# hamorrar/juicefs

Hardware: AMD Instinct MI355X
Metric: sealed+checksummed GB/s, 4 MiB blocks (higher is better)
Workload: dtype u8; 1 GPU; 64.0 GiB device-resident batch of 4 MiB blocks per GPU, aes256gcm seal + CRC32C full; blocks_per_gpu=16384, resident_blocks_per_gpu=16384, block_bytes=4194304, algo=aes256gcm, mode=seal, aes_kernel=ttable, engine=one process per GPU, parallelism=block-sharded x1, no collective

## Files before the change

### juicefs_amd/csrc/jfsx_dev.h

```cpp
#pragma once
#include "jfsx_internal.h"

namespace jfsx {

__device__ __forceinline__ uint32_t lds_u32(const char *lds, uint32_t byteaddr) {
    return *reinterpret_cast<const uint32_t *>(lds + byteaddr);
}
__device__ __forceinline__ uint4 lds_u4(const char *lds, uint32_t byteaddr) {
    return *reinterpret_cast<const uint4 *>(lds + byteaddr);
}

template <int K>
__device__ __forceinline__ uint32_t byte_x4(uint32_t x) {
    uint32_t r;
    if constexpr (K == 0)
        asm("v_lshlrev_b32_sdwa %0, 2, %1 dst_sel:DWORD dst_unused:UNUSED_PAD src0_sel:DWORD src1_sel:BYTE_0" : "=v"(r) : "v"(x));
    else if constexpr (K == 1)
        asm("v_lshlrev_b32_sdwa %0, 2, %1 dst_sel:DWORD dst_unused:UNUSED_PAD src0_sel:DWORD src1_sel:BYTE_1" : "=v"(r) : "v"(x));
    else if constexpr (K == 2)
        asm("v_lshlrev_b32_sdwa %0, 2, %1 dst_sel:DWORD dst_unused:UNUSED_PAD src0_sel:DWORD src1_sel:BYTE_2" : "=v"(r) : "v"(x));
    else
        asm("v_lshlrev_b32_sdwa %0, 2, %1 dst_sel:DWORD dst_unused:UNUSED_PAD src0_sel:DWORD src1_sel:BYTE_3" : "=v"(r) : "v"(x));
    return r;
}
#define CRC_T(t, x, k) lds_u32(lds, byte_x4<(k)>(x) + CB + 1024u * (t))

template <uint32_t CB, int S = 16>
__device__ __forceinline__ uint32_t crc_piece(const char *lds, uint32_t A, uint32_t p0, uint32_t p1, uint32_t p2,
                                              uint32_t p3) {
#define X3(a, b, c) __builtin_amdgcn_bitop3_b32((a), (b), (c), 0x96)
    uint32_t s = S < 0 ? A : X3(CRC_T(S, A, 0), CRC_T(S + 1, A, 1), CRC_T(S + 2, A, 2)) ^ CRC_T(S + 3, A, 3);
    uint32_t q = p0 ^ s;
    return X3(X3(X3(CRC_T(0, q, 0), CRC_T(1, q, 1), CRC_T(2, q, 2)), X3(CRC_T(3, q, 3), CRC_T(4, p1, 0), CRC_T(5, p1, 1)),
                 X3(CRC_T(6, p1, 2), CRC_T(7, p1, 3), CRC_T(8, p2, 0))),
              X3(CRC_T(9, p2, 1), CRC_T(10, p2, 2), CRC_T(11, p2, 3)),
              X3(CRC_T(12, p3, 0), CRC_T(13, p3, 1), X3(CRC_T(14, p3, 2), CRC_T(15, p3, 3), 0u)));
#undef X3
}

typedef __attribute__((address_space(1))) const uint32_t gcu32;
struct CrcL1Base {
    uint64_t a, b;
};
__device__ __forceinline__ CrcL1Base crc_l1_base(const uint32_t *gcrc) {
    CrcL1Base g = {(uint64_t)gcrc + 8192u, (uint64_t)gcrc + 12288u};
    asm volatile("" : "+s"(g.a), "+s"(g.b));
    return g;
}
template <int I>
__device__ __forceinline__ uint32_t crc_l1_term(const CrcL1Base &g, uint4 p) {
    const uint32_t w = I < 4 ? p.y : (I < 8 ? p.z : p.w);
    const uint32_t o = byte_x4<(I & 3)>(w);
    const __attribute__((address_space(1))) char *t = (const __attribute__((address_space(1))) char *)(I < 8 ? g.a : g.b);
    return *(gcu32 *)(t + o + (1024 * (4 + I) - (I < 8 ? 8192 : 12288)));
}

template <int S, int LG, int UR, int J = 0>
__device__ __forceinline__ void crc_l1_issue(const CrcL1Base &g, const uint4 (&d)[UR], uint32_t (&lv)[LG]) {
    if constexpr (J < LG) {
        lv[J] = crc_l1_term<LG * (S / UR) + J>(g, d[S % UR]);
        crc_l1_issue<S, LG, UR, J + 1>(g, d, lv);
    }
}

constexpr uint32_t kCrcbXl = 16 * 256;
__device__ __forceinline__ const uint32_t *crc_composed(const DevTables &tab) { return tab.crcx + kCrcxDwords; }
__device__ __forceinline__ uint32_t crc_xlb(const DevTables &tab, uint32_t l) {
    const uint32_t *b = crc_composed(tab) + kCrcbXl;
    asm volatile("" : "+s"(b));
    return b[l];
}
__device__ __forceinline__ uint32_t crc_xl(const DevTables &tab, uint32_t l) {
    const uint32_t *x = tab.crcx;
    asm volatile("" : "+s"(x));
    return x[l];
}
template <uint32_t CB>
__device__ __forceinline__ uint32_t crc_piece_b(const char *lds, uint32_t B, uint32_t p0, uint32_t L) {
    const uint32_t q = p0 ^ B;
    return __builtin_amdgcn_bitop3_b32(
        __builtin_amdgcn_bitop3_b32(CRC_T(0, q, 0), CRC_T(1, q, 1), CRC_T(2, q, 2), 0x96), CRC_T(3, q, 3), L, 0x96);
}
template <uint32_t CB>
__device__ __forceinline__ uint32_t crc_shift1008(const char *lds, uint32_t A) {
    return __builtin_amdgcn_bitop3_b32(CRC_T(16, A, 0), CRC_T(17, A, 1), CRC_T(18, A, 2), 0x96) ^ CRC_T(19, A, 3);
}

template <int CRCMODE>
__device__ __forceinline__ uint4 crc_src(uint4 c, uint4 p) {
    return (CRCMODE & 4) ? c : p;
}

template <uint32_t CB, int S = 16>
__device__ __noinline__ uint32_t crc_partial(const char *lds, uint32_t A, const uint32_t p[4], int n) {
    uint32_t c = S < 0 ? A : CRC_T(S, A, 0) ^ CRC_T(S + 1, A, 1) ^ CRC_T(S + 2, A, 2) ^ CRC_T(S + 3, A, 3);
    for (int i = 0; i < n; i++) {
        uint32_t byte = (p[i >> 2] >> (8 * (i & 3))) & 0xffu;
        c = lds_u32(lds, (((c ^ byte) & 0xffu) << 2) + CB + 1024u * 15) ^ (c >> 8);
    }
    return c;
}

typedef unsigned int v4u __attribute__((ext_vector_type(4)));
typedef __attribute__((address_space(1))) v4u gv4u;
__device__ __forceinline__ uint4 gld16(const uint8_t *p) {
    const v4u v = *(const gv4u *)(p);
    return make_uint4(v.x, v.y, v.z, v.w);
}
__device__ __forceinline__ uint4 gld16_nt(const uint8_t *p) {
    const v4u v = __builtin_nontemporal_load((const gv4u *)(p));
    return make_uint4(v.x, v.y, v.z, v.w);
}
__device__ __forceinline__ void gst16(uint8_t *p, uint4 v) {
    v4u w = {v.x, v.y, v.z, v.w};
    *(gv4u *)(p) = w;
}
__device__ __forceinline__ void gst16_nt(uint8_t *p, uint4 v) {
    v4u w = {v.x, v.y, v.z, v.w};
    __builtin_nontemporal_store(w, (gv4u *)(p));
}
template <int NT>
__device__ __forceinline__ uint4 ald16(const uint8_t *p) { return (NT & 1) ? gld16_nt(p) : gld16(p); }
template <int NT>
__device__ __forceinline__ void ast16(uint8_t *p, uint4 v) {
    if (NT & 2)
        gst16_nt(p, v);
    else
        gst16(p, v);
}

__device__ __forceinline__ uint4 load_piece(const uint8_t *src, uint64_t o, uint64_t end) {
    if (o + 16 <= end) return gld16(src + o);
    uint32_t w[4] = {0, 0, 0, 0};
    for (uint64_t i = o; i < end && i < o + 16; i++) w[(i - o) >> 2] |= (uint32_t)src[i] << (8 * ((i - o) & 3));
    return make_uint4(w[0], w[1], w[2], w[3]);
}

__device__ __forceinline__ void store_piece(uint8_t *dst, uint64_t o, uint64_t end, uint4 v) {
    if (o + 16 <= end) {
        gst16(dst + o, v);
        return;
    }
    uint32_t w[4] = {v.x, v.y, v.z, v.w};
    for (uint64_t i = o; i < end && i < o + 16; i++) dst[i] = (uint8_t)(w[(i - o) >> 2] >> (8 * ((i - o) & 3)));
}


__device__ __forceinline__ void crc_verify_block(const BlkDev &blk, BlkOut &o, uint32_t lane) {
    const uint64_t nseg = (blk.len + kSeg - 1) / kSeg;
    for (uint64_t base = 0; base < nseg; base += 64) {
        const uint64_t s = base + lane;
        bool bad = false;
        uint32_t got = 0, ex = 0;
        if (s < nseg) {
            got = blk.crc_calc[s];
            const uint8_t *e = blk.crc + 4 * s;
            ex = ((uint32_t)e[0] << 24) | ((uint32_t)e[1] << 16) | ((uint32_t)e[2] << 8) | e[3];
            bad = got != ex;
        }
        const uint64_t m = __ballot(bad);
        if (m) {
            const int first = __builtin_ctzll(m);
            const uint32_t g2 = __shfl(got, first, 64), e2 = __shfl(ex, first, 64);
            if (lane == 0) {
                o.bad_seg = (int32_t)(base + first);
                o.got = g2;
                o.expect = e2;
            }
            return;
        }
    }
}

}
```

### juicefs_amd/csrc/jfsx_gcm.hip

```cpp

#include "jfsx_dev.h"

#define JFSX_HD __device__ __forceinline__
#define BS3(a, b, c, tt) __builtin_amdgcn_bitop3_b32((a), (b), (c), (tt))
#define PERM(hi, lo, sel) __builtin_amdgcn_perm((hi), (lo), (sel))
#define OPAQUE(x)                                 \
    do {                                          \
        (x) = __builtin_amdgcn_readfirstlane(x);  \
        asm volatile("" : "+s"(x));               \
    } while (0)
#include "jfsx_aes_bs.h"

namespace jfsx {

constexpr int kAeadNt = 3;
constexpr uint32_t kLdsCrc = 0;
constexpr uint32_t kLdsTT = 20480;
constexpr uint32_t kLdsGh = 24576;
constexpr uint32_t kLdsAesOff = 24576;
constexpr uint32_t kLdsAes = 65536 + kLdsAesOff;
constexpr uint32_t kLdsBasis = kLdsAes + 65536;
constexpr uint32_t kLdsSegRaw = kLdsBasis + 2048;
constexpr uint32_t kLdsSegFlag = kLdsSegRaw + 512;
constexpr uint32_t kLdsP = kLdsSegFlag + 512;
constexpr uint32_t kLdsBytes = kLdsP + 4096 + 32;

__device__ __forceinline__ uint32_t rotl8(uint32_t x) { return __builtin_amdgcn_alignbit(x, x, 24); }
__device__ __forceinline__ uint32_t xor3(uint32_t a, uint32_t b, uint32_t c) {
    return __builtin_amdgcn_bitop3_b32(a, b, c, 0x96);
}
__device__ __forceinline__ uint32_t rk_load(const uint32_t *rk, int i) {
    uint32_t k = rk[i];
    if (i >= 8 && i < 56) {
        k = (k >> 8) | (k << 24);
        OPAQUE(k);
    }
    return k;
}

#define AES_SEL(k) (0x0c020000u | ((4u + (k)) << 8))
#define TA(w, k) lds_u32(lds, __builtin_amdgcn_perm((w), loff, AES_SEL(k)) + kLdsAesOff)
#define TB(w, k) lds_u32(lds, __builtin_amdgcn_perm((w), loff, AES_SEL(k)) + (kLdsAesOff + 128u))

#define AES_COL(o, i0, i1, i2, i3, rkv) \
    o = xor3(TA(i0, 0), TB(i2, 2), rotl8(xor3(TA(i1, 1), TB(i3, 3), (rkv))));
#define AES_ROUND(o0, o1, o2, o3, i0, i1, i2, i3, r) \
    AES_COL(o0, i0, i1, i2, i3, rk[4 * (r) + 0])     \
    AES_COL(o1, i1, i2, i3, i0, rk[4 * (r) + 1])     \
    AES_COL(o2, i2, i3, i0, i1, rk[4 * (r) + 2])     \
    AES_COL(o3, i3, i0, i1, i2, rk[4 * (r) + 3])

#define AES_LAST(o, a, b, c, d, rkv)                                                             \
    o = __builtin_amdgcn_bitop3_b32(                                                             \
            __builtin_amdgcn_bitop3_b32(TB(a, 0), TA(b, 1), 0xffu, 0xe4) ,       \
            __builtin_amdgcn_bitop3_b32(TA(c, 2), TB(d, 3), 0x00ff0000u, 0xe4),                 \
            0x0000ffffu, 0xe4) ^ (rkv);

template <int NS>
__device__ __forceinline__ void aes_ctr_blocks(const char *lds, uint32_t loff, const uint32_t *rk, const uint32_t *k1,
                                               const uint32_t (&ctr)[NS], uint32_t (&ks)[NS][4]) {
    uint32_t a[NS][4], b[NS][4];
#pragma unroll
    for (int s = 0; s < NS; s++) {
        const uint32_t x3 = __builtin_bswap32(ctr[s]) ^ rk[3];
        a[s][0] = k1[0] ^ rotl8(TB(x3, 3));
        a[s][1] = k1[1] ^ TB(x3, 2);
        a[s][2] = k1[2] ^ rotl8(TA(x3, 1));
        a[s][3] = k1[3] ^ TA(x3, 0);
    }
#pragma unroll
    for (int r = 2; r <= 13; r += 2) {
#pragma unroll
        for (int s = 0; s < NS; s++) { AES_ROUND(b[s][0], b[s][1], b[s][2], b[s][3], a[s][0], a[s][1], a[s][2], a[s][3], r); }
#pragma unroll
        for (int s = 0; s < NS; s++) { AES_ROUND(a[s][0], a[s][1], a[s][2], a[s][3], b[s][0], b[s][1], b[s][2], b[s][3], r + 1); }
    }
#pragma unroll
    for (int s = 0; s < NS; s++) {
        AES_LAST(ks[s][0], a[s][0], a[s][1], a[s][2], a[s][3], rk[56]);
        AES_LAST(ks[s][1], a[s][1], a[s][2], a[s][3], a[s][0], rk[57]);
        AES_LAST(ks[s][2], a[s][2], a[s][3], a[s][0], a[s][1], rk[58]);
        AES_LAST(ks[s][3], a[s][3], a[s][0], a[s][1], a[s][2], rk[59]);
    }
}

__device__ __forceinline__ void aes_r2_uniform(const char *lds, uint32_t loff, const uint32_t *rk, const uint32_t *k1,
                                               uint32_t U, uint32_t (&u)[4]) {
    const uint32_t x3 = __builtin_bswap32(U << 8) ^ rk[3];
    const uint32_t a1 = k1[1] ^ TB(x3, 2);
    const uint32_t a2 = k1[2] ^ rotl8(TA(x3, 1));
    const uint32_t a3 = k1[3] ^ TA(x3, 0);
    u[0] = xor3(TB(a2, 2), rotl8(xor3(TA(a1, 1), TB(a3, 3), rk[8])), 0u);
    u[1] = xor3(TA(a1, 0), TB(a3, 2), rotl8(TA(a2, 1) ^ rk[9]));
    u[2] = xor3(TA(a2, 0), rotl8(xor3(TA(a3, 1), TB(a1, 3), rk[10])), 0u);
    u[3] = xor3(TA(a3, 0), TB(a1, 2), rotl8(TB(a2, 3) ^ rk[11]));
}

__device__ __forceinline__ uint4 aes_r2_entry(const char *lds, uint32_t loff, uint32_t rk3, uint32_t k10, uint32_t c) {
    const uint32_t x3 = (c << 24) ^ rk3;
    const uint32_t a0 = k10 ^ rotl8(TB(x3, 3));
    return make_uint4(TA(a0, 0), rotl8(TB(a0, 3)), TB(a0, 2), rotl8(TA(a0, 1)));
}

template <int I>
struct AesStep {
    static constexpr int value = I;
};
struct AesNoSide {
    template <int I>
    __device__ __forceinline__ void operator()(AesStep<I>) const {}
};
template <int NS, class Side>
__device__ __forceinline__ void aes_rounds_3_14(const char *lds, uint32_t loff, const uint32_t *rk,
                                                uint32_t (&b)[NS][4], uint32_t (&ks)[NS][4], const Side &side) {
    uint32_t a[NS][4];
    side(AesStep<0>());
#pragma unroll
    for (int s = 0; s < NS; s++) { AES_ROUND(a[s][0], a[s][1], a[s][2], a[s][3], b[s][0], b[s][1], b[s][2], b[s][3], 3); }
    side(AesStep<1>());
#define JFSX_AES_PAIR(r)                                                                                                \
    _Pragma("unroll") for (int s = 0; s < NS; s++) {                                                                    \
        AES_ROUND(b[s][0], b[s][1], b[s][2], b[s][3], a[s][0], a[s][1], a[s][2], a[s][3], r);                           \
    }                                                                                                                   \
    side(AesStep<(r) - 2>());                                                                                           \
    _Pragma("unroll") for (int s = 0; s < NS; s++) {                                                                    \
        AES_ROUND(a[s][0], a[s][1], a[s][2], a[s][3], b[s][0], b[s][1], b[s][2], b[s][3], (r) + 1);                     \
    }                                                                                                                   \
    side(AesStep<(r) - 1>());
    JFSX_AES_PAIR(4)
    JFSX_AES_PAIR(6)
    JFSX_AES_PAIR(8)
    JFSX_AES_PAIR(10)
    JFSX_AES_PAIR(12)
#undef JFSX_AES_PAIR
#pragma unroll
    for (int s = 0; s < NS; s++) {
        AES_LAST(ks[s][0], a[s][0], a[s][1], a[s][2], a[s][3], 0u);
        AES_LAST(ks[s][1], a[s][1], a[s][2], a[s][3], a[s][0], 0u);
        AES_LAST(ks[s][2], a[s][2], a[s][3], a[s][0], a[s][1], 0u);
        AES_LAST(ks[s][3], a[s][3], a[s][0], a[s][1], a[s][2], 0u);
    }
}

template <int NS, class Side = AesNoSide>
__device__ __forceinline__ void aes_ctr_blocks_u(const char *lds, uint32_t loff, const uint32_t *rk,
                                                 const uint32_t *k1, const uint32_t (&ctr)[NS],
                                                 const uint32_t (&u)[NS][4], const uint32_t (&du)[NS][4],
                                                 const uint32_t (&cym)[NS], uint32_t (&ks)[NS][4],
                                                 const Side &side = Side()) {
    uint32_t b[NS][4];
#define UC(t, w) (__builtin_amdgcn_bitop3_b32((t), cym[s], du[s][w], 0x78) ^ u[s][w])
#pragma unroll
    for (int s = 0; s < NS; s++) {
        const uint4 pe = lds_u4(lds, ((ctr[s] << 4) & 0xff0u) + kLdsP);
        b[s][0] = UC(pe.x, 0);
        b[s][1] = UC(pe.y, 1);
        b[s][2] = UC(pe.z, 2);
        b[s][3] = UC(pe.w, 3);
    }
#undef UC
    aes_rounds_3_14<NS>(lds, loff, rk, b, ks, side);
}

template <int Q, class Side>
__device__ __forceinline__ void aes_ctr_blocks_p(const char *lds, uint32_t loff, const uint32_t *rk, uint32_t pb,
                                                 const uint32_t (&u)[4], const uint32_t (&du)[4], uint32_t cy3,
                                                 uint32_t (&ks)[2][4], const Side &side) {
    uint32_t b[2][4];
#pragma unroll
    for (int s = 0; s < 2; s++) {
        const uint4 pe = lds_u4(lds, pb + 1024u * (Q + s));
        const uint32_t t[4] = {pe.x, pe.y, pe.z, pe.w};
#pragma unroll
        for (int w = 0; w < 4; w++)
            b[s][w] = Q + s == 3 ? __builtin_amdgcn_bitop3_b32(t[w], cy3, du[w], 0x78) ^ u[w] : t[w] ^ u[w];
    }
    aes_rounds_3_14<2>(lds, loff, rk, b, ks, side);
}

struct GhLane {
    uint32_t sel[4];
    uint32_t off[4];
    bool r1, r2;
    uint32_t p1, p2;
};

__device__ __forceinline__ GhLane gh_lane(uint32_t lane) {
    GhLane g;
    const uint32_t q = lane & 15, k = q >> 2;
#pragma unroll
    for (int bb = 0; bb < 4; bb++) g.sel[bb] = 0x0c0c0000u | ((4u + ((bb + q) & 3)) << 8) | (uint32_t)bb;
#pragma unroll
    for (int dd = 0; dd < 4; dd++) {
        uint32_t o = 0;
#pragma unroll
        for (int bb = 0; bb < 4; bb++) {
            const uint32_t j = 4 * ((dd + k) & 3) + ((bb + q) & 3);
            o |= (j << 4) << (8 * bb);
        }
        g.off[dd] = o;
    }
    g.r1 = (k & 1) != 0;
    g.r2 = (k & 2) != 0;
    g.p1 = g.r1 ? 0x07060504u : 0x03020100u;
    g.p2 = g.r2 ? 0x07060504u : 0x03020100u;
    return g;
}

__device__ __forceinline__ void gh_rho(const uint32_t a[4], const GhLane &g, uint32_t R[4]) {
    uint32_t u[4];
#pragma unroll
    for (int i = 0; i < 4; i++) u[i] = PERM(a[(i + 2) & 3], a[i], g.p2);
#pragma unroll
    for (int i = 0; i < 4; i++) R[i] = PERM(u[(i + 1) & 3], u[i], g.p1);
}
__device__ __forceinline__ void gh_rho_inv(const uint32_t R[4], const GhLane &g, uint32_t a[4]) {
    uint32_t u[4];
#pragma unroll
    for (int i = 0; i < 4; i++) u[i] = g.r1 ? R[(i + 3) & 3] : R[i];
#pragma unroll
    for (int i = 0; i < 4; i++) a[i] = g.r2 ? u[(i + 2) & 3] : u[i];
}

__device__ __forceinline__ void ghash_step(const char *lds, uint32_t R[4], const GhLane &g, uint4 c) {
#if JFSX_GH8 == 4
    uint32_t S[4] = {c.x, c.y, c.z, c.w};
#pragma unroll
    for (int h = 0; h < 4; h++) {
        uint4 t[4];
#pragma unroll
        for (int q = 0; q < 4; q++) t[q] = lds_u4(lds, kLdsGh + __builtin_amdgcn_perm(R[h], g.off[h], g.sel[q]));
#define GX(f, i) S[i] = xor3(xor3(t[0].f, t[1].f, t[2].f), t[3].f, S[i])
        GX(x, 0); GX(y, 1); GX(z, 2); GX(w, 3);
#undef GX
        __builtin_amdgcn_sched_barrier(0);
    }
#elif JFSX_GH8
    uint32_t S[4] = {c.x, c.y, c.z, c.w};
#pragma unroll
    for (int h = 0; h < 2; h++) {
        uint4 t[8];
#pragma unroll
        for (int q = 0; q < 8; q++) {
            const int dd = 2 * h + (q >> 2), bb = q & 3;
            t[q] = lds_u4(lds, kLdsGh + __builtin_amdgcn_perm(R[dd], g.off[dd], g.sel[bb]));
        }
#define GX(f, i) S[i] = xor3(xor3(t[0].f, t[1].f, t[2].f), xor3(t[3].f, t[4].f, t[5].f), xor3(t[6].f, t[7].f, S[i]))
        GX(x, 0); GX(y, 1); GX(z, 2); GX(w, 3);
#undef GX
        __builtin_amdgcn_sched_barrier(0);
    }
#else
    uint4 t[16];
#pragma unroll
    for (int dd = 0; dd < 4; dd++)
#pragma unroll
        for (int bb = 0; bb < 4; bb++)
            t[4 * dd + bb] = lds_u4(lds, kLdsGh + __builtin_amdgcn_perm(R[dd], g.off[dd], g.sel[bb]));
#define GX(f, cf) xor3(xor3(xor3(t[0].f, t[1].f, t[2].f), xor3(t[3].f, t[4].f, t[5].f), xor3(t[6].f, t[7].f, t[8].f)), \
                       xor3(t[9].f, t[10].f, t[11].f), xor3(xor3(t[12].f, t[13].f, t[14].f), t[15].f, cf))
    const uint32_t S[4] = {GX(x, c.x), GX(y, c.y), GX(z, c.z), GX(w, c.w)};
#undef GX
#endif
    gh_rho(S, g, R);
}

struct Stream {
    uint64_t sub0, sub1;
    uint32_t acc[4];
    uint64_t jlast;
    bool has;
    uint32_t A, lend;
    uint64_t seg0;
};

__device__ __forceinline__ void crc_share(char *lds, uint32_t slot, uint32_t raw) {
    atomicXor(reinterpret_cast<uint32_t *>(lds + kLdsSegRaw) + slot, raw);
    reinterpret_cast<uint32_t *>(lds + kLdsSegFlag)[slot] = 1u;
}

template <int CRCMODE>
__device__ __forceinline__ void crc_segment_done(const BlkDev &blk, const DevTables &tab, uint32_t lane, uint32_t xl,
                                                 uint64_t seg0, uint32_t A, bool partial, char *lds, uint64_t c0) {
    const uint32_t raw = wave_xor(crc_mulmod(xl, A));
    if (lane == 0) {
        if (partial) {
            crc_share(lds, (uint32_t)((seg0 - c0) / kSeg), raw);
            return;
        }
        const uint32_t crc = ~(tab.crcx[96] ^ raw);
        const uint64_t si = seg0 / kSeg;
        if ((CRCMODE & 3) == 1)
            *reinterpret_cast<uint32_t *>(blk.crc + 4 * si) = __builtin_bswap32(crc);
        else
            blk.crc_calc[si] = crc;
    }
}

template <int CRCMODE>
__device__ __noinline__ void crc_segment_end(const BlkDev &blk, const DevTables &tab, uint32_t lane, uint32_t xl,
                                             uint64_t seg0, uint64_t seg1, uint32_t A, uint32_t lend,
                                             uint64_t tailRef, bool partial, char *lds, uint32_t slot) {
    const uint32_t Lseg = (uint32_t)(seg1 - seg0);
    uint32_t v;
    if (lend == 0) {
        const uint32_t sh = tailRef == seg1 ? xl : crc_mulmod(crc_xpow8_fast((uint32_t)(seg1 - tailRef), tab.crcx), xl);
        v = crc_mulmod(sh, A);
    } else {
        v = crc_mulmod(crc_xpow8_fast(Lseg - lend, tab.crcx), A);
    }
    const uint32_t raw = wave_xor(v);
    if (lane == 0) {
        if (partial) {
            crc_share(lds, slot, raw);
            return;
        }
        const uint32_t K = Lseg == (uint32_t)kSeg ? tab.crcx[96] : crc_mulmod(crc_xpow8_fast(Lseg, tab.crcx), 0xffffffffu);
        const uint32_t crc = ~(K ^ raw);
        const uint64_t si = seg0 / kSeg;
        if ((CRCMODE & 3) == 1)
            *reinterpret_cast<uint32_t *>(blk.crc + 4 * si) = __builtin_bswap32(crc);
        else
            blk.crc_calc[si] = crc;
    }
}

template <bool OPEN, int CRCMODE>
__device__ __noinline__ Stream row_generic(char *lds, uint32_t loff, const GhLane gl, const GcmSched *sch,
                                           const BlkDev blk, const DevTables tab, uint32_t lane, uint32_t xl, Stream st,
                                           uint64_t row, uint64_t c0, uint64_t c1) {
    uint32_t rk[60];
#pragma unroll
    for (int i = 0; i < 60; i++) rk[i] = rk_load(sch->rk, i);
    const uint32_t k1[4] = {sch->k1[0], sch->k1[1], sch->k1[2], sch->k1[3]};
    const uint64_t o = row + 16 * lane;
    const uint64_t end = st.sub1;
    const bool valid = o < end, full = o + 16 <= end;
    uint4 d = load_piece(blk.src, o, end);
    const uint32_t ctr[1] = {(uint32_t)((o >> 4) + 2)};
    uint32_t ks[1][4];
    aes_ctr_blocks<1>(lds, loff, rk, k1, ctr, ks);
    uint4 x = make_uint4(d.x ^ ks[0][0], d.y ^ ks[0][1], d.z ^ ks[0][2], d.w ^ ks[0][3]);
    uint4 c = OPEN ? d : x, p = OPEN ? x : d;
    if (!full) {
        const int nv = valid ? (int)(end - o) : 0;
        uint32_t m[4];
        for (int k = 0; k < 4; k++) {
            int bytes = nv - 4 * k;
            m[k] = bytes >= 4 ? 0xffffffffu : (bytes <= 0 ? 0u : ((1u << (8 * bytes)) - 1u));
        }
        c.x &= m[0]; c.y &= m[1]; c.z &= m[2]; c.w &= m[3];
        p.x &= m[0]; p.y &= m[1]; p.z &= m[2]; p.w &= m[3];
    }
    if (valid) store_piece(blk.dst, o, end, OPEN ? p : c);
    uint32_t t[4] = {st.acc[0], st.acc[1], st.acc[2], st.acc[3]};
    ghash_step(lds, t, gl, c);
    if (valid) {
        st.acc[0] = t[0]; st.acc[1] = t[1]; st.acc[2] = t[2]; st.acc[3] = t[3];
        st.jlast = o >> 4;
        st.has = true;
    }
    const uint4 cq = crc_src<CRCMODE>(c, p);
    if (CRCMODE) {
        if (full) {
            st.A = crc_piece<kLdsCrc>(lds, st.A, cq.x, cq.y, cq.z, cq.w);
            st.lend = (uint32_t)(o + 16 - st.seg0);
        } else if (valid) {
            const uint32_t pw[4] = {cq.x, cq.y, cq.z, cq.w};
            st.A = crc_partial<kLdsCrc>(lds, st.A, pw, (int)(end - o));
            st.lend = (uint32_t)(end - st.seg0);
        }
        const uint64_t seg1 = st.seg0 + kSeg < c1 ? st.seg0 + kSeg : c1;
        if (row + 1024 >= seg1) {
            crc_segment_end<CRCMODE>(blk, tab, lane, xl, st.seg0, seg1, st.A, st.lend, row, st.seg0 < st.sub0, lds,
                                     (uint32_t)((st.seg0 - c0) / kSeg));
            st.A = 0;
            st.lend = 0;
            st.seg0 = seg1;
        }
    }
    return st;
}

template <bool BS>
struct GcmShape {
    static constexpr uint32_t waves = BS ? 8u : (uint32_t)kWaves;
    static constexpr uint32_t threads = waves * 64u;
};

#ifdef JFSX_KS_PHASES
__device__ unsigned long long g_main_ts[8];
#define MAIN_STAMP(cond, i)                                                                  \
    do {                                                                                     \
        __syncthreads();                                                                     \
        if ((cond) && threadIdx.x == 0) g_main_ts[i] = __builtin_amdgcn_s_memrealtime(); \
    } while (0)
#else
#define MAIN_STAMP(cond, i) ((void)0)
#endif

#ifdef JFSX_ABLATE_TRACE
__device__ uint64_t g_wgtrace[4 * 65536];
#endif

template <bool OPEN, int CRCMODE, bool BS, int KL1>
__device__ __forceinline__ void gcm_task(char *lds, const Task task, const BlkDev *__restrict__ blks,
                                         const GcmSched *__restrict__ sched, uint32_t *__restrict__ partial,
                                         uint32_t *__restrict__ pexp, const DevTables &tab, uint32_t tid,
                                         uint32_t wave, uint32_t lane, uint32_t loff, const GhLane &gl, uint32_t xl) {
#ifdef JFSX_ABLATE_TRACE
    const uint64_t trace_t0 = __builtin_amdgcn_s_memrealtime();
#endif
    const BlkDev blk = blks[task.blk];
    const GcmSched *sch = sched + task.blk;
    if (tid < 128)
        reinterpret_cast<uint4 *>(lds + kLdsBasis)[tid] = reinterpret_cast<const uint4 *>(sch->basis)[tid];
    if (tid < 256) reinterpret_cast<uint32_t *>(lds + kLdsSegRaw)[tid] = 0u;
    if (wave < 4) {
        uint32_t c = (wave << 6) | lane;
        asm volatile("" : "+v"(c));
        const uint4 e = aes_r2_entry(lds, loff, sch->rk[3], sch->k1[0], c);
        reinterpret_cast<uint4 *>(lds + kLdsP)[c] = e;
        if constexpr (!BS) {
            if (c < 2) reinterpret_cast<uint4 *>(lds + kLdsP)[256 + c] = e;
        }
    }
    __syncthreads();
    {
        uint4 *lg = reinterpret_cast<uint4 *>(lds + kLdsGh);
        const uint4 *lb = reinterpret_cast<const uint4 *>(lds + kLdsBasis);
#ifdef JFSX_ABLATE_GHBUILD
        if (false)
#endif
        for (uint32_t u = tid; u < 1024; u += GcmShape<BS>::threads) {
            const uint32_t j = u & 15, blow = u >> 4;
            uint4 z = make_uint4(0, 0, 0, 0);
#pragma unroll
            for (int k = 2; k < 8; k++) {
                if ((blow >> (7 - k)) & 1) {
                    const uint4 v = lb[8 * j + k];
                    z.x ^= v.x; z.y ^= v.y; z.z ^= v.z; z.w ^= v.w;
                }
            }
            const uint4 h0 = lb[8 * j], h1 = lb[8 * j + 1];
            lg[(blow << 4) | j] = z;
            lg[((blow | 64) << 4) | j] = make_uint4(z.x ^ h1.x, z.y ^ h1.y, z.z ^ h1.z, z.w ^ h1.w);
            lg[((blow | 128) << 4) | j] = make_uint4(z.x ^ h0.x, z.y ^ h0.y, z.z ^ h0.z, z.w ^ h0.w);
            lg[((blow | 192) << 4) | j] =
                make_uint4(z.x ^ h0.x ^ h1.x, z.y ^ h0.y ^ h1.y, z.z ^ h0.z ^ h1.z, z.w ^ h0.w ^ h1.w);
        }
    }
    __syncthreads();

    const bool first_task = task.blk == 0 && task.c0 == 0;
    MAIN_STAMP(first_task, 2);
    const uint64_t c0 = task.c0, c1 = task.c1;
    const uint32_t nseg = (uint32_t)((c1 - c0 + kSeg - 1) / kSeg);
    constexpr uint32_t V = GcmShape<BS>::waves;

    constexpr bool kRowSplit = !BS;
    Stream st;
    if (kRowSplit) {
        const uint32_t npairs = (uint32_t)((c1 - c0 + 2047) / 2048);
        const uint32_t ra = 2 * (wave * npairs / V), rb = 2 * ((wave + 1) * npairs / V);
        st.sub0 = c0 + (uint64_t)ra * 1024;
        st.sub1 = rb > ra ? (c0 + (uint64_t)rb * 1024 < c1 ? c0 + (uint64_t)rb * 1024 : c1) : st.sub0;
    } else {
        const uint32_t sa = wave * nseg / V, sb = (wave + 1) * nseg / V;
        st.sub0 = c0 + (uint64_t)sa * kSeg;
        st.sub1 = sb > sa ? (c0 + (uint64_t)sb * kSeg < c1 ? c0 + (uint64_t)sb * kSeg : c1) : st.sub0;
    }
    st.acc[0] = st.acc[1] = st.acc[2] = st.acc[3] = 0;
    st.jlast = 0;
    st.has = false;
    st.A = 0;
    st.lend = 0;
    st.seg0 = c0 + (st.sub0 - c0) / kSeg * kSeg;
    const bool act = st.sub1 > st.sub0;
    const uint64_t fr = (st.sub1 - st.sub0) / 1024;
    const uint64_t rf = act ? fr : 0;
    const uint64_t ld0 = st.sub0;
    const uint8_t *src = blk.src;
    uint8_t *dst = blk.dst;
    const uint64_t lo = 16 * lane;

    uint64_t r0 = 0;
    if (BS && act && rf >= 32) {
        const uint64_t nfs = rf / 32;
        const uint32_t nrk[3] = {sch->c012[0], sch->c012[1], sch->c012[2]};
        const uint32_t rk3 = sch->rk[3];
        constexpr int PF = 4;
        uint4 pf[PF];
#pragma unroll
        for (int q = 0; q < PF; q++) pf[q] = ald16<kAeadNt>(src + ld0 + 1024 * q + lo);
        for (uint64_t sg = 0; sg < nfs; sg++) {
            const uint64_t base = ld0 + (uint64_t)kSeg * sg;
            uint32_t ks[128];
            jfsx_bs::ctr32(ks, nrk, rk3, (uint32_t)((base >> 4) + lane + 2),
                           [&](int r, int w) { return sch->bsu[r][w]; }, sch->r1c);
            const bool more = sg + 1 < nfs;
#pragma unroll
            for (int k = 0; k < 32; k++) {
                const uint4 d = pf[k % PF];
                const uint64_t o = base + 1024 * k + lo;
                if (k + PF < 32 || more) pf[k % PF] = ald16<kAeadNt>(src + o + 1024 * PF);
                const uint4 x = make_uint4(d.x ^ ks[k], d.y ^ ks[32 + k], d.z ^ ks[64 + k], d.w ^ ks[96 + k]);
                const uint4 c = OPEN ? d : x, p = OPEN ? x : d;
                ast16<kAeadNt>(dst + o, OPEN ? p : c);
                const uint4 cq = crc_src<CRCMODE>(c, p);
                ghash_step(lds, st.acc, gl, c);
                if (CRCMODE) st.A = crc_piece<kLdsCrc>(lds, st.A, cq.x, cq.y, cq.z, cq.w);
            }
            if (CRCMODE) {
                crc_segment_done<CRCMODE>(blk, tab, lane, xl, st.seg0, st.A, false, lds, c0);
                st.A = 0;
                st.seg0 += kSeg;
            }
        }
        r0 = 32 * nfs;
    }
    uint32_t rk[60];
#pragma unroll
    for (int i = 0; i < 60; i++) rk[i] = rk_load(sch->rk, i);
    uint32_t k1[4] = {sch->k1[0], sch->k1[1], sch->k1[2], sch->k1[3]};
    uint4 nxt = r0 < rf ? ald16<kAeadNt>(src + ld0 + 1024 * r0 + lo) : make_uint4(0, 0, 0, 0);
    constexpr int UR = 2;
    constexpr bool kL1 = KL1 > 0 && kRowSplit && CRCMODE != 0 && OPEN == ((CRCMODE & 4) != 0);
    constexpr bool kPeriod = !BS;
    auto xl_here = [&]() { return kL1 ? crc_xl(tab, lane) : xl; };
    static_assert(!kL1 || KL1 == 12, "B form: TT_4..15 are in the L1 image only");
    bool bform = false;
    if (act && rf >= r0 + UR) {
        uint4 nn[UR];
#pragma unroll
        for (int u = 0; u < UR; u++) nn[u] = ald16<kAeadNt>(src + ld0 + 1024 * (r0 + u) + lo);
        uint32_t uw[4] = {0, 0, 0, 0};
        uint32_t uw0 = 0;
        bool uwok = false;
        const uint32_t rb0 = (uint32_t)((ld0 - c0) >> 10) / 2u * 2u;
        const CrcL1Base l1g = kL1 ? crc_l1_base(crc_composed(tab)) : CrcL1Base{0, 0};
        auto two_rows = [&]() __attribute__((always_inline)) {
            uint4 dd[UR];
#pragma unroll
            for (int u = 0; u < UR; u++) dd[u] = nn[u];
            const uint64_t o0 = ld0 + 1024 * r0 + lo;
            if (!kL1 && r0 + 2 * UR - 1 < rf) {
#pragma unroll
                for (int u = 0; u < UR; u++) nn[u] = ald16<kAeadNt>(src + o0 + 1024 * (UR + u));
            }
            constexpr int LG = kL1 ? JFSX_CRC_L1LG : 1, LLAG = JFSX_CRC_L1LAG, LSTEPS = kL1 ? UR * KL1 / LG : 0;
            static_assert(!kL1 || (KL1 % LG == 0 && LSTEPS + LLAG <= 12),
                          "the gathers, their folds and the prefetch must fit the 12 round groups");
            uint32_t crcL[UR], lv[LSTEPS ? LSTEPS : 1][LG];
#pragma unroll
            for (int u = 0; u < UR; u++) crcL[u] = 0;
            const bool pre = r0 + 2 * UR - 1 < rf;
            auto side = [&](auto step) {
                if constexpr (kL1) {
                    constexpr int S = decltype(step)::value;
                    __builtin_amdgcn_sched_barrier(0);
                    if constexpr (S >= LLAG && S - LLAG < LSTEPS) {
                        constexpr int F = S - LLAG;
                        uint32_t t = crcL[F % UR];
#pragma unroll
                        for (int j = 0; j + 1 < LG; j += 2) t = xor3(t, lv[F][j], lv[F][j + 1]);
                        if (LG & 1) t ^= lv[F][LG - 1];
                        crcL[F % UR] = t;
                    }
                    if constexpr (S < LSTEPS) {
                        crc_l1_issue<S, LG, UR>(l1g, dd, lv[S]);
                    } else if constexpr (S == LSTEPS) {
                        if (pre) {
#pragma unroll
                            for (int u = 0; u < UR; u++) nn[u] = ald16<kAeadNt>(src + o0 + 1024 * (UR + u));
                        }
                    }
                    __builtin_amdgcn_sched_barrier(0);
                }
            };
            uint32_t ctrs[UR];
#pragma unroll
            for (int u = 0; u < UR; u++) ctrs[u] = (uint32_t)((o0 >> 4) + 2 + 64 * u);
            uint32_t ks2[UR][4];
            {
                uint32_t C = (uint32_t)(((ld0 + 1024 * r0) >> 4) + 2);
                OPAQUE(C);
                if (!uwok || (C >> 8) < uw0 || ((C + 64u * UR + 63u) >> 8) - uw0 > 63u) {
                    uw0 = C >> 8;
                    aes_r2_uniform(lds, loff, rk, k1, uw0 + lane, uw);
                    uwok = true;
                }
                uint32_t u2[UR][4], d2[UR][4], cym[UR];
#pragma unroll
                for (int u = 0; u < UR; u++) {
                    const uint32_t Cr = C + 64u * u;
                    const uint32_t i0 = (Cr >> 8) - uw0;
                    cym[u] = (uint32_t)__builtin_amdgcn_sbfe((int)((Cr & 255u) + lane), 8, 1);
#pragma unroll
// ... 666 lines not shown
```

Before: 942.6 GB/s.

## Software-pipeline AES rounds across two rows with sched barriers, use global address-space loads

Restructures the AES rounds 3-14 into separate issue (LDS table lookups) and finish (xor/rotate combine) phases. The two row states are interleaved so one row's lookups are in flight while the other row's previous round is combined, with sched_barrier fences pinning that order. It also casts CRC table reads and CRC stores to address_space(1) pointers so the compiler emits global rather than flat memory instructions. The rigid schedule raises register pressure (two 16-entry temporaries) and blocks compiler reordering, and it now requires NS==2.

```diff
diff --git a/juicefs_amd/csrc/jfsx_dev.h b/juicefs_amd/csrc/jfsx_dev.h
--- a/juicefs_amd/csrc/jfsx_dev.h
+++ b/juicefs_amd/csrc/jfsx_dev.h
@@ -68,12 +68,12 @@
 __device__ __forceinline__ uint32_t crc_xlb(const DevTables &tab, uint32_t l) {
     const uint32_t *b = crc_composed(tab) + kCrcbXl;
     asm volatile("" : "+s"(b));
-    return b[l];
+    return *(gcu32 *)(b + l);
 }
 __device__ __forceinline__ uint32_t crc_xl(const DevTables &tab, uint32_t l) {
     const uint32_t *x = tab.crcx;
     asm volatile("" : "+s"(x));
-    return x[l];
+    return *(gcu32 *)(x + l);
 }
 template <uint32_t CB>
 __device__ __forceinline__ uint32_t crc_piece_b(const char *lds, uint32_t B, uint32_t p0, uint32_t L) {
diff --git a/juicefs_amd/csrc/jfsx_gcm.hip b/juicefs_amd/csrc/jfsx_gcm.hip
--- a/juicefs_amd/csrc/jfsx_gcm.hip
+++ b/juicefs_amd/csrc/jfsx_gcm.hip
@@ -110,36 +110,77 @@
     template <int I>
     __device__ __forceinline__ void operator()(AesStep<I>) const {}
 };
+__device__ __forceinline__ void aes_issue(const char *lds, uint32_t loff, const uint32_t (&x)[4], uint32_t (&t)[16]) {
+#pragma unroll
+    for (int c = 0; c < 4; c++) {
+        t[4 * c + 0] = TA(x[c], 0);
+        t[4 * c + 1] = TB(x[(c + 2) & 3], 2);
+        t[4 * c + 2] = TA(x[(c + 1) & 3], 1);
+        t[4 * c + 3] = TB(x[(c + 3) & 3], 3);
+    }
+}
+__device__ __forceinline__ void aes_finish(const uint32_t (&t)[16], const uint32_t *rk, int r, uint32_t (&x)[4]) {
+#pragma unroll
+    for (int c = 0; c < 4; c++) x[c] = xor3(t[4 * c], t[4 * c + 1], rotl8(xor3(t[4 * c + 2], t[4 * c + 3], rk[4 * r + c])));
+}
+__device__ __forceinline__ void aes_issue_last(const char *lds, uint32_t loff, const uint32_t (&x)[4],
+                                               uint32_t (&t)[16]) {
+#pragma unroll
+    for (int c = 0; c < 4; c++) {
+        t[4 * c + 0] = TB(x[c], 0);
+        t[4 * c + 1] = TA(x[(c + 1) & 3], 1);
+        t[4 * c + 2] = TA(x[(c + 2) & 3], 2);
+        t[4 * c + 3] = TB(x[(c + 3) & 3], 3);
+    }
+}
+__device__ __forceinline__ void aes_finish_last(const uint32_t (&t)[16], uint32_t (&ks)[4]) {
+#pragma unroll
+    for (int c = 0; c < 4; c++)
+        ks[c] = __builtin_amdgcn_bitop3_b32(__builtin_amdgcn_bitop3_b32(t[4 * c], t[4 * c + 1], 0xffu, 0xe4),
+                                            __builtin_amdgcn_bitop3_b32(t[4 * c + 2], t[4 * c + 3], 0x00ff0000u, 0xe4),
+                                            0x0000ffffu, 0xe4);
+}
+
 template <int NS, class Side>
 __device__ __forceinline__ void aes_rounds_3_14(const char *lds, uint32_t loff, const uint32_t *rk,
-                                                uint32_t (&b)[NS][4], uint32_t (&ks)[NS][4], const Side &side) {
-    uint32_t a[NS][4];
+                                                uint32_t (&x)[NS][4], uint32_t (&ks)[NS][4], const Side &side) {
+    static_assert(NS == 2, "a row pair");
+    uint32_t t[2][16];
+#define JFSX_PART() __builtin_amdgcn_sched_barrier(0)
     side(AesStep<0>());
-#pragma unroll
-    for (int s = 0; s < NS; s++) { AES_ROUND(a[s][0], a[s][1], a[s][2], a[s][3], b[s][0], b[s][1], b[s][2], b[s][3], 3); }
-    side(AesStep<1>());
-#define JFSX_AES_PAIR(r)                                                                                                \
-    _Pragma("unroll") for (int s = 0; s < NS; s++) {                                                                    \
-        AES_ROUND(b[s][0], b[s][1], b[s][2], b[s][3], a[s][0], a[s][1], a[s][2], a[s][3], r);                           \
-    }                                                                                                                   \
-    side(AesStep<(r) - 2>());                                                                                           \
-    _Pragma("unroll") for (int s = 0; s < NS; s++) {                                                                    \
-        AES_ROUND(a[s][0], a[s][1], a[s][2], a[s][3], b[s][0], b[s][1], b[s][2], b[s][3], (r) + 1);                     \
-    }                                                                                                                   \
-    side(AesStep<(r) - 1>());
-    JFSX_AES_PAIR(4)
-    JFSX_AES_PAIR(6)
-    JFSX_AES_PAIR(8)
-    JFSX_AES_PAIR(10)
-    JFSX_AES_PAIR(12)
-#undef JFSX_AES_PAIR
-#pragma unroll
-    for (int s = 0; s < NS; s++) {
-        AES_LAST(ks[s][0], a[s][0], a[s][1], a[s][2], a[s][3], 0u);
-        AES_LAST(ks[s][1], a[s][1], a[s][2], a[s][3], a[s][0], 0u);
-        AES_LAST(ks[s][2], a[s][2], a[s][3], a[s][0], a[s][1], 0u);
-        AES_LAST(ks[s][3], a[s][3], a[s][0], a[s][1], a[s][2], 0u);
-    }
+    JFSX_PART();
+    aes_issue(lds, loff, x[0], t[0]);
+    JFSX_PART();
+    aes_issue(lds, loff, x[1], t[1]);
+    JFSX_PART();
+    aes_finish(t[0], rk, 3, x[0]);
+    JFSX_PART();
+#define JFSX_AES_GROUP(r, ISSUE, FINISH0)    \
+    side(AesStep<(r) - 3>());                \
+    ISSUE(lds, loff, x[0], t[0]);            \
+    JFSX_PART();                             \
+    aes_finish(t[1], rk, (r) - 1, x[1]);     \
+    JFSX_PART();                             \
+    ISSUE(lds, loff, x[1], t[1]);            \
+    JFSX_PART();                             \
+    FINISH0;                                 \
+    JFSX_PART();
+#define JFSX_AES_FULL(r) JFSX_AES_GROUP(r, aes_issue, aes_finish(t[0], rk, r, x[0]))
+    JFSX_AES_FULL(4)
+    JFSX_AES_FULL(5)
+    JFSX_AES_FULL(6)
+    JFSX_AES_FULL(7)
+    JFSX_AES_FULL(8)
+    JFSX_AES_FULL(9)
+    JFSX_AES_FULL(10)
+    JFSX_AES_FULL(11)
+    JFSX_AES_FULL(12)
+    JFSX_AES_FULL(13)
+    JFSX_AES_GROUP(14, aes_issue_last, aes_finish_last(t[0], ks[0]))
+    aes_finish_last(t[1], ks[1]);
+#undef JFSX_AES_FULL
+#undef JFSX_AES_GROUP
+#undef JFSX_PART
 }
 
 template <int NS, class Side = AesNoSide>
@@ -290,10 +331,11 @@
         }
         const uint32_t crc = ~(tab.crcx[96] ^ raw);
         const uint64_t si = seg0 / kSeg;
+        typedef __attribute__((address_space(1))) uint32_t gu32;
         if ((CRCMODE & 3) == 1)
-            *reinterpret_cast<uint32_t *>(blk.crc + 4 * si) = __builtin_bswap32(crc);
+            *(gu32 *)(blk.crc + 4 * si) = __builtin_bswap32(crc);
         else
-            blk.crc_calc[si] = crc;
+            *(gu32 *)(blk.crc_calc + si) = crc;
     }
 }
 
```

After: 948.9 GB/s, median of 6. About the same (+0.7%).
